# Breakthrough/PySceneDetect

Measured on NVIDIA H100. Metric: frames/sec scored (1080p, ContentDetector), higher is better.
Workload: dtype u8

## Files before the change

### pyscenedetect_b200/csrc/hsv_half2.cuh

```cuda
#pragma once

#include <cuda_fp16.h>
#include <stdint.h>

namespace psd {

struct Px16 {
    uint32_t h[4], s[4], v[4];
};

__device__ __forceinline__ uint32_t y_px(uint32_t b, uint32_t g, uint32_t r) {
    return (r * 4899u + g * 9617u + b * 1868u + 8192u) >> 14;
}

__host__ __device__ constexpr uint32_t y_coef_word(int word, int k0, int which) {
    uint32_t r = 0;
    for (int b = 0; b < 4; ++b) {
        const int g = 4 * word + b - k0;
        uint32_t c = 0;
        if (g == 0) c = which ? 7u : 76u;
        if (g == 1) c = which ? 37u : 145u;
        if (g == 2) c = which ? 19u : 35u;
        r |= c << (8 * b);
    }
    return r;
}

template <int P>
__device__ __forceinline__ uint32_t y_of_pixel(const uint32_t (&w)[12]) {
    constexpr int k0 = 3 * P, j0 = k0 >> 2, j1 = (k0 + 2) >> 2;
    uint32_t lo = __dp4a(w[j0], y_coef_word(j0, k0, 0), 8192u);
    uint32_t hi = __dp4a(w[j0], y_coef_word(j0, k0, 1), 0u);
    if (j1 != j0) {
        lo = __dp4a(w[j1], y_coef_word(j1, k0, 0), lo);
        hi = __dp4a(w[j1], y_coef_word(j1, k0, 1), hi);
    }
    return (hi * 256u + lo) >> 14;
}

__device__ __forceinline__ uint32_t byte_of(const uint32_t (&w)[12], int k) {
    return (w[k >> 2] >> ((k & 3) * 8)) & 0xFFu;
}

struct LutView7 {
    uint32_t cs;
    uint32_t ch;
};

__device__ __forceinline__ LutView7 make_lut7(uint32_t lut_smem_addr, int lane) {
    LutView7 l;
    l.cs = lut_smem_addr + (uint32_t)lane * 4u - 0x6400u * 128u;
    l.ch = lut_smem_addr + 32768u + (uint32_t)lane * 4u;
    return l;
}

__device__ __forceinline__ void lut_fill7(float* lut, int tid, int nthreads) {
    for (int t = tid; t < 512; t += nthreads) {
        const int row = t >> 1, which = t & 1;
        float v = 0.0f;
        if (row) {
            const int q = which ? __double2int_rn(737280.0 / (6.0 * (double)row))
                                : __double2int_rn(1044480.0 / (double)row);
            v = (float)q * 0.000244140625f;
        }
        float4* dst = reinterpret_cast<float4*>(lut + which * 8192 + row * 32);
#pragma unroll
        for (int j = 0; j < 8; ++j) dst[j] = make_float4(v, v, v, v);
    }
}

namespace v7 {

__device__ __forceinline__ __half2 as_h2(uint32_t u) { return *reinterpret_cast<__half2*>(&u); }
__device__ __forceinline__ uint32_t as_u32(__half2 h) { return *reinterpret_cast<uint32_t*>(&h); }

__device__ __forceinline__ uint32_t hsub2u(uint32_t a, uint32_t b) { return as_u32(__hsub2(as_h2(a), as_h2(b))); }
__device__ __forceinline__ uint32_t hfma2u(uint32_t a, uint32_t b, uint32_t c) {
    return as_u32(__hfma2(as_h2(a), as_h2(b), as_h2(c)));
}
__device__ __forceinline__ uint32_t heq2m(uint32_t a, uint32_t b) { return __heq2_mask(as_h2(a), as_h2(b)); }
__device__ __forceinline__ uint32_t bitsel(uint32_t m, uint32_t x, uint32_t y) {
    uint32_t r;
    asm("lop3.b32 %0, %1, %2, %3, 0xCA;" : "=r"(r) : "r"(m), "r"(x), "r"(y));
    return r;
}
__device__ __forceinline__ uint32_t even_bytes_magic(uint32_t t) {
    uint32_t r;
    asm("lop3.b32 %0, %1, 0x00FF00FF, %2, 0xEA;" : "=r"(r) : "r"(t), "r"(0x64006400u));
    return r;
}
__device__ __forceinline__ float lds(uint32_t addr) {
    float r;
    asm volatile("ld.shared.f32 %0, [%1];" : "=f"(r) : "r"(addr));
    return r;
}
__device__ __forceinline__ float fma_rz_(float a, float b, float c) {
    float r;
    asm("fma.rz.f32 %0, %1, %2, %3;" : "=f"(r) : "f"(a), "f"(b), "f"(c));
    return r;
}
__device__ __forceinline__ float fma_rm_(float a, float b, float c) {
    float r;
    asm("fma.rm.f32 %0, %1, %2, %3;" : "=f"(r) : "f"(a), "f"(b), "f"(c));
    return r;
}

struct PairOut7 {
    uint32_t yh0, yh1, ys0, ys1;
    uint32_t vh;
};

__device__ __forceinline__ void pair(uint32_t Bh, uint32_t Gh, uint32_t Rh, const LutView7& lut, PairOut7& o) {
    const uint32_t Vh = __vimax3_u16x2(Bh, Gh, Rh);
    const uint32_t mh = __vimin3_u16x2(Bh, Gh, Rh);
    const uint32_t dh = hsub2u(Vh, mh);
    const uint32_t di = Vh - mh;
    const uint32_t hR = hsub2u(Gh, Bh);
    const uint32_t hG = hfma2u(dh, 0x40004000u, hsub2u(Bh, Rh));
    const uint32_t hB = hfma2u(dh, 0x44004400u, hsub2u(Rh, Gh));
    const uint32_t eR = heq2m(Vh, Rh);
    const uint32_t eG = heq2m(Vh, Gh);
    const uint32_t hh = bitsel(eR, hR, bitsel(eG, hG, hB));
    const float d0 = __low2float(as_h2(dh)), d1 = __high2float(as_h2(dh));
    const float h0 = __low2float(as_h2(hh)), h1 = __high2float(as_h2(hh));
    const uint32_t aS0 = __dp2a_lo(Vh, 0x00000080u, lut.cs), aS1 = __dp2a_lo(Vh, 0x00008000u, lut.cs);
    const uint32_t aH0 = __dp2a_lo(di, 0x00000080u, lut.ch), aH1 = __dp2a_lo(di, 0x00008000u, lut.ch);
    o.ys0 = __float_as_uint(fma_rz_(d0, lds(aS0), 32768.5f));
    o.ys1 = __float_as_uint(fma_rz_(d1, lds(aS1), 32768.5f));
    o.yh0 = __float_as_uint(fma_rm_(h0, lds(aH0), 49152.5f));
    o.yh1 = __float_as_uint(fma_rm_(h1, lds(aH1), 49152.5f));
    o.vh = Vh;
}

__device__ __forceinline__ uint32_t fix_hue4(uint32_t hw) {
    uint32_t m;
    asm("lop3.b32 %0, %1, %2, 0x80808080, 0x80;" : "=r"(m) : "r"(hw), "r"(hw + hw));
    return hw - (m >> 7) * 76u;
}

}

__device__ __forceinline__ void hsv16_v7(const uint32_t (&w)[12], Px16& o, const LutView7& lut) {
    const uint32_t K = 0x64646464u;
#pragma unroll
    for (int g = 0; g < 4; ++g) {
        const uint32_t wa = w[3 * g], wb = w[3 * g + 1], wc = w[3 * g + 2];
        const uint32_t B01 = __byte_perm(wa, K, 0x4340);
        const uint32_t t01 = __byte_perm(wa, wb, 0x5421);
        const uint32_t G01 = v7::even_bytes_magic(t01);
        const uint32_t R01 = __byte_perm(t01, K, 0x4341);
        const uint32_t R23 = __byte_perm(wc, K, 0x4340);
        const uint32_t t23 = __byte_perm(wb, wc, 0x6532);
        const uint32_t B23 = v7::even_bytes_magic(t23);
        const uint32_t G23 = __byte_perm(t23, K, 0x4341);
        v7::PairOut7 p, q;
        v7::pair(B01, G01, R01, lut, p);
        v7::pair(B23, G23, R23, lut, q);
        const uint32_t hw = __byte_perm(__byte_perm(p.yh0, p.yh1, 0x0051), __byte_perm(q.yh0, q.yh1, 0x0051), 0x5410);
        o.h[g] = v7::fix_hue4(hw);
        o.s[g] = __byte_perm(__byte_perm(p.ys0, p.ys1, 0x0051), __byte_perm(q.ys0, q.ys1, 0x0051), 0x5410);
        o.v[g] = __byte_perm(p.vh, q.vh, 0x6420);
    }
}

}
```

### pyscenedetect_b200/csrc/score_kernel.cu

```cuda
#include "hsv_half2.cuh"
#include "psd_common.cuh"

namespace psd {

constexpr int kPxPerThread = 16;

__device__ __forceinline__ uint32_t smem_u32(const void* p) {
    return (uint32_t)__cvta_generic_to_shared(p);
}
__device__ __forceinline__ void mbar_init(unsigned long long* bar, uint32_t count) {
    asm volatile("mbarrier.init.shared::cta.b64 [%0], %1;" ::"r"(smem_u32(bar)), "r"(count));
}
__device__ __forceinline__ void mbar_expect_tx(unsigned long long* bar, uint32_t bytes) {
    asm volatile("mbarrier.arrive.expect_tx.shared::cta.b64 _, [%0], %1;" ::"r"(smem_u32(bar)),
                 "r"(bytes)
                 : "memory");
}
__device__ __forceinline__ void bulk_g2s(void* dst, const void* src, uint32_t bytes,
                                         unsigned long long* bar) {
    asm volatile(
        "cp.async.bulk.shared::cluster.global.mbarrier::complete_tx::bytes [%0], [%1], %2, [%3];" ::
            "r"(smem_u32(dst)),
        "l"(src), "r"(bytes), "r"(smem_u32(bar))
        : "memory");
}

constexpr int kWsConsumerWarps = 24;
constexpr int kWsConsumers = kWsConsumerWarps * 32;
constexpr int kWsStages = 4;
constexpr int kWsSideWarps = kWsStages;
constexpr int kWsThreads = kWsConsumers + kWsSideWarps * 32;
static_assert(kWsSideWarps == 4 && kWsConsumerWarps % 4 == 0, "one side warp per SM sub-partition");
constexpr int kWsUnroll = 4;
constexpr int kWsStripPx = kWsConsumers * kPxPerThread;
constexpr int kWsStripBytes = kWsStripPx * 3;
static_assert(kWsStages % kWsUnroll == 0, "the stage ring must be a whole number of loop bodies");

struct __align__(128) WsSmem {
    uint8_t ring[kWsStages][kWsStripBytes];
    float lut[256 * 64];
    unsigned long long full[kWsStages];
    unsigned long long empty[kWsStages];
    uint32_t accl[kWsStages][4][32];
    uint32_t accl_sink[kWsStages][4][32];
    uint32_t yhist[kWsStages][256];
    uint32_t vhist[kWsStages][256];
};

__device__ __forceinline__ uint32_t sad4_acc(uint32_t a, uint32_t b, uint32_t c) {
    uint32_t r;
    asm volatile("vabsdiff4.u32.u32.u32.add %0, %1, %2, %3;" : "=r"(r) : "r"(a), "r"(b), "r"(c));
    return r;
}
template <int OFF>
__device__ __forceinline__ void mbar_wait_hint_off(uint32_t bar, uint32_t parity) {
    asm volatile(
        "{\n\t"
        ".reg .pred p;\n\t"
        "WAIT_%=:\n\t"
        "mbarrier.try_wait.parity.shared::cta.b64 p, [%0+%3], %1, %2;\n\t"
        "@p bra DONE_%=;\n\t"
        "bra WAIT_%=;\n\t"
        "DONE_%=:\n\t"
        "}" ::"r"(bar),
        "r"(parity), "r"(20000u), "n"(OFF)
        : "memory");
}
__device__ __forceinline__ void mbar_wait_hint(unsigned long long* bar, uint32_t parity) {
    mbar_wait_hint_off<0>(smem_u32(bar), parity);
}
template <int OFF>
__device__ __forceinline__ void lds128_off(uint32_t addr, uint32_t& x, uint32_t& y, uint32_t& z, uint32_t& w) {
    asm volatile("ld.shared.v4.u32 {%0,%1,%2,%3}, [%4+%5];" : "=r"(x), "=r"(y), "=r"(z), "=r"(w) : "r"(addr), "n"(OFF));
}
template <int OFF>
__device__ __forceinline__ void red_shared_add_off(uint32_t addr, uint32_t v) {
    asm volatile("red.shared.add.u32 [%0+%2], %1;" ::"r"(addr), "r"(v), "n"(OFF) : "memory");
}
template <int OFF>
__device__ __forceinline__ void mbar_arrive_off(uint32_t bar) {
    asm volatile("mbarrier.arrive.shared::cta.b64 _, [%0+%1];" ::"r"(bar), "n"(OFF) : "memory");
}

__host__ __device__ __forceinline__ int chunk_first(int c, int n_frames, int n_chunks) {
    return (int)(((long long)c * n_frames) / n_chunks);
}
struct WsItem {
    int f0, nf;
    int px0, valid_px;
    int it_begin;
    int slots;
    int walked;
};
__device__ __forceinline__ WsItem ws_item(const ScoreArgs& a, int item) {
    WsItem w;
    const int chunk = item % a.n_chunks;
    const int strip = item / a.n_chunks;
    w.f0 = chunk_first(chunk, a.n_frames, a.n_chunks);
    w.nf = chunk_first(chunk + 1, a.n_frames, a.n_chunks) - w.f0;
    w.px0 = strip * kWsStripPx;
    w.valid_px = min(kWsStripPx, a.n_pixels - w.px0) & ~15;
    const bool have_halo = (a.features & PSD_F_HSV) && (w.f0 > 0 || a.prev != nullptr);
    w.it_begin = have_halo ? 0 : 1;
    w.walked = w.nf + 1 - w.it_begin;
    w.slots = (w.walked + kWsUnroll - 1) / kWsUnroll * kWsUnroll;
    return w;
}

struct WsAddr {
    uint32_t ring;
    uint32_t full;
    uint32_t acc;
};

template <uint32_t F, int J>
__device__ __forceinline__ void ws_step(const ScoreArgs& a, WsSmem& sm, const WsAddr& ad, uint32_t parity, int stage0,
                                        uint32_t sad_acc, bool mine, int fi, int my_px, int lane, uint32_t zero,
                                        const LutView7& lut7, const Px16& prev, Px16& cur) {
    constexpr bool kHSV = (F & PSD_F_HSV) != 0;
    constexpr bool kSUM = (F & PSD_F_BGRSUM) != 0;
    constexpr bool kYH = (F & PSD_F_YHIST) != 0;
    constexpr bool kEDGE = (F & PSD_F_EDGES) != 0;
    if (kHSV) {
        if ((J & 1) == 0) {
            mbar_wait_hint_off<J * 8>(ad.full, parity);
            mbar_wait_hint_off<J * 8 + 8>(ad.full, parity);
        }
    } else {
        mbar_wait_hint_off<J * 8>(ad.full, parity);
    }
    uint32_t w[12];
    lds128_off<J * kWsStripBytes>(ad.ring, w[0], w[1], w[2], w[3]);
    lds128_off<J * kWsStripBytes + 16>(ad.ring, w[4], w[5], w[6], w[7]);
    lds128_off<J * kWsStripBytes + 32>(ad.ring, w[8], w[9], w[10], w[11]);
    if (kHSV) {
        hsv16_v7(w, cur, lut7);
        uint32_t sad_h = sad4_acc(cur.h[0], prev.h[0], zero), sad_s = sad4_acc(cur.s[0], prev.s[0], zero),
                 sad_v = sad4_acc(cur.v[0], prev.v[0], zero);
#pragma unroll
        for (int j = 1; j < 4; ++j) {
            sad_h = sad4_acc(cur.h[j], prev.h[j], sad_h);
            sad_s = sad4_acc(cur.s[j], prev.s[j], sad_s);
            sad_v = sad4_acc(cur.v[j], prev.v[j], sad_v);
        }
        red_shared_add_off<J * 512>(sad_acc, sad_h);
        red_shared_add_off<J * 512 + 128>(sad_acc, sad_s);
        red_shared_add_off<J * 512 + 256>(sad_acc, sad_v);
        if (kEDGE && mine) {
            uint8_t* vp = a.vplane + (int64_t)fi * a.n_pixels + my_px;
            if ((a.n_pixels & 15) == 0) {
                *reinterpret_cast<uint4*>(vp) = make_uint4(cur.v[0], cur.v[1], cur.v[2], cur.v[3]);
            } else {
                for (int p = 0; p < kPxPerThread; ++p) vp[p] = (uint8_t)(cur.v[p >> 2] >> ((p & 3) * 8));
            }
            const uint32_t vh = smem_u32(sm.vhist[stage0 + J]);
#pragma unroll
            for (int p = 0; p < kPxPerThread; ++p)
                red_shared_add_off<0>(__dp4a(cur.v[p >> 2], 4u << ((p & 3) * 8), vh), 1u);
        }
    }
    if (mine) {
        if (kSUM) {
            uint32_t bsum = 0;
#pragma unroll
            for (int j = 0; j < 12; ++j) bsum = __dp4a(w[j], 0x01010101u, bsum);
            red_shared_add_off<J * 512 + 384>(ad.acc, bsum);
        }
        if (kYH) {
            uint32_t* hist = sm.yhist[stage0 + J];
#define PSD_YH(i) atomicAdd(&hist[y_of_pixel<i>(w)], 1u);
            PSD_YH(0) PSD_YH(1) PSD_YH(2) PSD_YH(3) PSD_YH(4) PSD_YH(5) PSD_YH(6) PSD_YH(7)
            PSD_YH(8) PSD_YH(9) PSD_YH(10) PSD_YH(11) PSD_YH(12) PSD_YH(13) PSD_YH(14) PSD_YH(15)
#undef PSD_YH
        }
    }
    if (lane == 0) mbar_arrive_off<kWsStages * 8 + J * 8>(ad.full);
}

template <int J>
__device__ __forceinline__ void ws_null_step(const WsAddr& ad, uint32_t parity, int lane) {
    mbar_wait_hint_off<J * 8>(ad.full, parity);
    if (lane == 0) mbar_arrive_off<kWsStages * 8 + J * 8>(ad.full);
}

template <uint32_t F>
__global__ void __launch_bounds__(kWsThreads, 1) psd_score_ws_kernel(const ScoreArgs a) {
    extern __shared__ __align__(128) uint8_t smem_raw[];
    WsSmem& sm = *reinterpret_cast<WsSmem*>(smem_raw);
    constexpr bool kHSV = (F & PSD_F_HSV) != 0;
    constexpr bool kSUM = (F & PSD_F_BGRSUM) != 0;
    constexpr bool kYH = (F & PSD_F_YHIST) != 0;
    constexpr bool kEDGE = (F & PSD_F_EDGES) != 0;
    constexpr int U = kWsUnroll;

    const int tid = threadIdx.x;
    const int lane = tid & 31;
    const int n_items = a.n_chunks * a.n_strips;

    for (int i = tid; i < kWsStages * 256; i += kWsThreads) {
        (&sm.yhist[0][0])[i] = 0;
        (&sm.vhist[0][0])[i] = 0;
    }
    for (int i = tid; i < kWsStages * 4 * 32; i += kWsThreads) {
        (&sm.accl[0][0][0])[i] = 0;
        (&sm.accl_sink[0][0][0])[i] = 0;
    }
    if (kHSV) lut_fill7(sm.lut, tid, kWsThreads);
    if (tid == 0) {
        for (int s = 0; s < kWsStages; ++s) {
            mbar_init(&sm.full[s], 1);
            mbar_init(&sm.empty[s], kWsConsumerWarps);
        }
        asm volatile("fence.mbarrier_init.release.cluster;" ::: "memory");
    }
    __syncthreads();

    if (tid >= kWsConsumers) {
        struct Cursor {
            int item, slot;
            WsItem w;
        };
        const int rs = (tid - kWsConsumers) >> 5;
        auto load = [&](Cursor& c) { if (c.item < n_items) c.w = ws_item(a, c.item); };
        auto advance = [&](Cursor& c) {
            c.slot += kWsStages;
            if (c.slot >= c.w.slots) { c.slot = rs; c.item += gridDim.x; load(c); }
        };
        auto issue = [&](Cursor& c) {
            if (lane == 0) {
                if (c.slot < c.w.walked) {
                    const int fi = c.w.f0 - 1 + c.w.it_begin + c.slot;
                    const uint8_t* src = (fi < 0 ? a.prev : a.frames + (int64_t)fi * a.frame_stride) + (int64_t)c.w.px0 * 3;
                    const uint32_t bytes = (uint32_t)c.w.valid_px * 3u;
                    mbar_expect_tx(&sm.full[rs], bytes);
                    bulk_g2s(sm.ring[rs], src, bytes, &sm.full[rs]);
                } else {
                    mbar_arrive_off<0>(smem_u32(&sm.full[rs]));
                }
            }
            advance(c);
        };
        Cursor ret{(int)blockIdx.x, rs, {}};
        load(ret);
        Cursor iss = ret;
        issue(iss);
        uint32_t parity = 0;
        while (ret.item < n_items) {
            mbar_wait_hint(&sm.empty[rs], parity);
            const int it = ret.w.it_begin + ret.slot;
            const bool real = ret.slot < ret.w.walked;
            const bool own = real && it >= 1;
            const int fi = ret.w.f0 - 1 + it;
            uint32_t tot[4] = {0u, 0u, 0u, 0u};
            if (own && (kHSV || kSUM)) {
#pragma unroll
                for (int c = 0; c < 4; ++c) {
                    if ((c < 3 && kHSV) || (c == 3 && kSUM)) {
                        tot[c] = sm.accl[rs][c][lane];
                        sm.accl[rs][c][lane] = 0;
                    }
                }
            }
            if (own) {
                if (kYH) {
#pragma unroll
                    for (int b = lane; b < 256; b += 32) {
                        const uint32_t v = sm.yhist[rs][b];
                        if (v) { sm.yhist[rs][b] = 0; atomicAdd(&a.yhist[(int64_t)fi * 256 + b], v); }
                    }
                }
                if (kEDGE) {
#pragma unroll
                    for (int b = lane; b < 256; b += 32) {
                        const uint32_t v = sm.vhist[rs][b];
                        if (v) { sm.vhist[rs][b] = 0; atomicAdd(&a.vhist[(int64_t)fi * 256 + b], v); }
                    }
                }
                if (ret.item < a.n_chunks && lane == 0)
                    a.sums[fi].has_prev = (fi > 0 || a.prev != nullptr) ? 1ull : 0ull;
            }
            __syncwarp();
            if (iss.item < n_items) issue(iss);
            if (own && (kHSV || kSUM)) {
#pragma unroll
                for (int c = 0; c < 4; ++c) {
                    if ((c < 3 && !kHSV) || (c == 3 && !kSUM)) continue;
                    const uint32_t v = __reduce_add_sync(0xFFFFFFFFu, tot[c]);
                    if (lane == 0 && v)
                        atomicAdd(reinterpret_cast<unsigned long long*>(&a.sums[fi]) + (c < 3 ? c : 4),
                                  (unsigned long long)v);
                }
            }
            advance(ret);
            parity ^= 1u;
        }
        return;
    }

    const LutView7 lut7 = make_lut7(smem_u32(sm.lut), lane);
    const uint32_t zero = a.shift24 ^ 0x01000000u;
    const uint32_t ring0 = smem_u32(sm.ring[0]) + tid * 48;
    const uint32_t full0 = smem_u32(&sm.full[0]);
    const uint32_t accl0 = smem_u32(&sm.accl[0][0][lane]);
    const uint32_t sink0 = smem_u32(&sm.accl_sink[0][0][lane]);
    int stage0 = 0;
    uint32_t parity = 0;
    WsAddr ad{ring0, full0, 0u};
    auto next_body = [&](uint32_t acc0) {
        stage0 += U;
        if (stage0 == kWsStages) {
            stage0 = 0;
            parity ^= 1u;
            ad.ring = ring0; ad.full = full0; ad.acc = acc0;
        } else {
            ad.ring += U * kWsStripBytes; ad.full += U * 8; ad.acc += U * 512;
        }
    };
    for (int item = blockIdx.x; item < n_items; item += gridDim.x) {
        const WsItem wi = ws_item(a, item);
        const int my_px = wi.px0 + tid * kPxPerThread;
        const bool active = tid * kPxPerThread < wi.valid_px;
        const uint32_t acc0 = active ? accl0 : sink0;
        ad.acc = acc0 + stage0 * 512;
        Px16 P0, P1;
#pragma unroll
        for (int j = 0; j < 4; ++j) P0.h[j] = P0.s[j] = P0.v[j] = P1.h[j] = P1.s[j] = P1.v[j] = 0;
        const int n = wi.walked;
        const int fbase = wi.f0 - 1 + wi.it_begin;
        int k = 0;
        uint32_t acc_first = sink0 + stage0 * 512;
#pragma unroll 1
        for (; k + U <= n; k += U) {
            const bool first_mine = active && (wi.it_begin + k >= 1);
            ws_step<F, 0>(a, sm, ad, parity, stage0, acc_first, first_mine, fbase + k, my_px, lane, zero, lut7, P0, P1);
            ws_step<F, 1>(a, sm, ad, parity, stage0, ad.acc, active, fbase + k + 1, my_px, lane, zero, lut7, P1, P0);
            ws_step<F, 2>(a, sm, ad, parity, stage0, ad.acc, active, fbase + k + 2, my_px, lane, zero, lut7, P0, P1);
            ws_step<F, 3>(a, sm, ad, parity, stage0, ad.acc, active, fbase + k + 3, my_px, lane, zero, lut7, P1, P0);
            next_body(acc0);
            acc_first = ad.acc;
        }
        if (k < n) {
            const int r = n - k;
            ws_step<F, 0>(a, sm, ad, parity, stage0, acc_first, active && (wi.it_begin + k >= 1), fbase + k, my_px,
                              lane, zero, lut7, P0, P1);
            if (r > 1) ws_step<F, 1>(a, sm, ad, parity, stage0, ad.acc, active, fbase + k + 1, my_px, lane, zero, lut7, P1, P0);
            else ws_null_step<1>(ad, parity, lane);
            if (r > 2) ws_step<F, 2>(a, sm, ad, parity, stage0, ad.acc, active, fbase + k + 2, my_px, lane, zero, lut7, P0, P1);
            else ws_null_step<2>(ad, parity, lane);
            ws_null_step<3>(ad, parity, lane);
            next_body(acc0);
        }
    }
}

static int pick_chunks(int n_frames, int n_strips, int grid) {
    long long best_cost = -1;
    int best = 1;
    const int c_max = n_frames < 4096 ? n_frames : 4096;
    for (int c = 1; c <= c_max; ++c) {
        const int longest = (n_frames + c - 1) / c;
        if (longest < 8 && c > 1) break;
        const long long per_cta = ((long long)n_strips * c + grid - 1) / grid;
        const long long cost = per_cta * (longest + 1);
        if (best_cost < 0 || cost < best_cost) { best_cost = cost; best = c; }
    }
    return best;
}

template <uint32_t F>
static int launch_ws(ScoreArgs a, int n_ws_strips, cudaStream_t stream) {
    const int smem = (int)sizeof(WsSmem);
    static int sm_count = 0;
    if (sm_count == 0) {
        int dev = 0;
        PSD_CUDA(cudaGetDevice(&dev));
        PSD_CUDA(cudaDeviceGetAttribute(&sm_count, cudaDevAttrMultiProcessorCount, dev));
    }
    PSD_CUDA(cudaFuncSetAttribute(psd_score_ws_kernel<F>, cudaFuncAttributeMaxDynamicSharedMemorySize, smem));
    a.shift24 = 0x01000000u;
    a.features = F;
    a.n_strips = n_ws_strips;
    a.n_chunks = pick_chunks(a.n_frames, n_ws_strips, sm_count);
    if (a.n_chunks > a.n_frames) a.n_chunks = a.n_frames;
    const int64_t items = (int64_t)a.n_chunks * n_ws_strips;
    PSD_REQUIRE(items > 0 && items < 2147483647LL, "score work items out of range (%lld)", (long long)items);
    const int grid = (int)(items < sm_count ? items : sm_count);
    psd_score_ws_kernel<F><<<grid, kWsThreads, smem, stream>>>(a);
    PSD_CHECK_LAUNCH();
    count_launch();
    return PSD_OK;
}

static int dispatch_ws(const ScoreArgs& a, uint32_t f, int n_ws_strips, cudaStream_t s) {
    switch (f & 15u) {
#define CASE(F) case F: return launch_ws<F>(a, n_ws_strips, s);
        CASE(1) CASE(2) CASE(3) CASE(4) CASE(5) CASE(6) CASE(7)
        CASE(9) CASE(11) CASE(13) CASE(15)
#undef CASE
        default:
            set_error("unsupported feature mask 0x%x", f);
            return PSD_ERR_INVALID;
    }
}

constexpr int kTailThreads = 128;
constexpr int kLutBytes = 256 * 64 * 4;

__device__ __forceinline__ void load_tail(const uint8_t* src, int n_bytes, uint32_t (&w)[12]) {
#pragma unroll
    for (int j = 0; j < 12; ++j) w[j] = 0;
#pragma unroll
    for (int k = 0; k < 48; ++k)
        if (k < n_bytes) w[k >> 2] |= (uint32_t)src[k] << ((k & 3) * 8);
}

__global__ void __launch_bounds__(kTailThreads) psd_score_tail_kernel(const ScoreArgs a) {
    extern __shared__ __align__(128) float lut[];
    const bool hsv = (a.features & PSD_F_HSV) != 0;
    if (hsv) lut_fill7(lut, threadIdx.x, blockDim.x);
    __syncthreads();
    const int fi = blockIdx.x * blockDim.x + threadIdx.x;
    if (fi >= a.n_frames) return;
    const int p16 = a.n_pixels & ~15, n = a.n_pixels - p16;
    const uint8_t* prev = fi > 0 ? a.frames + (int64_t)(fi - 1) * a.frame_stride : a.prev;
    uint32_t w[12];
    load_tail(a.frames + (int64_t)fi * a.frame_stride + (int64_t)p16 * 3, 3 * n, w);
    unsigned long long* sums = reinterpret_cast<unsigned long long*>(&a.sums[fi]);
    if (hsv) {
        const LutView7 lut7 = make_lut7(smem_u32(lut), threadIdx.x & 31);
        Px16 cur;
        hsv16_v7(w, cur, lut7);
        if (prev) {
            uint32_t wp[12];
            load_tail(prev + (int64_t)p16 * 3, 3 * n, wp);
            Px16 pre;
            hsv16_v7(wp, pre, lut7);
            uint32_t sad_h = 0, sad_s = 0, sad_v = 0;
#pragma unroll
            for (int j = 0; j < 4; ++j) {
                sad_h = __vsadu4(cur.h[j], pre.h[j]) + sad_h;
                sad_s = __vsadu4(cur.s[j], pre.s[j]) + sad_s;
                sad_v = __vsadu4(cur.v[j], pre.v[j]) + sad_v;
            }
            atomicAdd(sums + 0, (unsigned long long)sad_h);
            atomicAdd(sums + 1, (unsigned long long)sad_s);
            atomicAdd(sums + 2, (unsigned long long)sad_v);
        }
        if (a.features & PSD_F_EDGES) {
            uint8_t* vp = a.vplane + (int64_t)fi * a.n_pixels + p16;
            for (int p = 0; p < n; ++p) {
                const uint32_t v = (cur.v[p >> 2] >> ((p & 3) * 8)) & 0xFFu;
                vp[p] = (uint8_t)v;
                atomicAdd(&a.vhist[(int64_t)fi * 256 + v], 1u);
            }
        }
    }
    if (a.features & PSD_F_BGRSUM) {
        uint32_t bsum = 0;
#pragma unroll
        for (int j = 0; j < 12; ++j) bsum = __dp4a(w[j], 0x01010101u, bsum);
        atomicAdd(sums + 4, (unsigned long long)bsum);
    }
    if (a.features & PSD_F_YHIST) {
        for (int p = 0; p < n; ++p)
            atomicAdd(&a.yhist[(int64_t)fi * 256 + y_px(byte_of(w, 3 * p), byte_of(w, 3 * p + 1), byte_of(w, 3 * p + 2))],
                      1u);
    }
    if (p16 == 0) a.sums[fi].has_prev = (fi > 0 || a.prev != nullptr) ? 1ull : 0ull;
}

static int launch_tail(ScoreArgs a, uint32_t features, cudaStream_t stream) {
    PSD_CUDA(cudaFuncSetAttribute(psd_score_tail_kernel, cudaFuncAttributeMaxDynamicSharedMemorySize, kLutBytes));
    a.features = features;
    const int grid = (a.n_frames + kTailThreads - 1) / kTailThreads;
    psd_score_tail_kernel<<<grid, kTailThreads, (features & PSD_F_HSV) ? kLutBytes : 0, stream>>>(a);
    PSD_CHECK_LAUNCH();
    count_launch();
    return PSD_OK;
}

int launch_score(const ScoreArgs& a, uint32_t features, cudaStream_t stream) {
    if (features & PSD_F_EDGES) features |= PSD_F_HSV;
    PSD_REQUIRE(a.n_frames > 0 && a.n_pixels > 0, "empty score launch");
    const uintptr_t al = reinterpret_cast<uintptr_t>(a.frames) | (uintptr_t)a.frame_stride |
                         reinterpret_cast<uintptr_t>(a.prev);
    PSD_REQUIRE((al & 15) == 0, "score pass input is not 16-byte aligned");
    const int p16 = a.n_pixels & ~15;
    if (p16 > 0) {
        const int rc = dispatch_ws(a, features, (p16 + kWsStripPx - 1) / kWsStripPx, stream);
        if (rc) return rc;
    }
    if (p16 < a.n_pixels) return launch_tail(a, features, stream);
    return PSD_OK;
}

__global__ void psd_test_hsv_kernel(const uint8_t* bgr, int64_t n_groups, uint8_t* h, uint8_t* s,
                                    uint8_t* v, uint8_t* y) {
    extern __shared__ __align__(128) float lutmem[];
    lut_fill7(lutmem, threadIdx.x, blockDim.x);
    const LutView7 lut7 = make_lut7(smem_u32(lutmem), threadIdx.x & 31);
    __syncthreads();
    for (int64_t g = blockIdx.x * (int64_t)blockDim.x + threadIdx.x; g < n_groups;
         g += (int64_t)gridDim.x * blockDim.x) {
        uint32_t w[12];
        const uint4* p = reinterpret_cast<const uint4*>(bgr + g * 48);
        const uint4 q0 = p[0], q1 = p[1], q2 = p[2];
        w[0] = q0.x; w[1] = q0.y; w[2] = q0.z; w[3] = q0.w;
        w[4] = q1.x; w[5] = q1.y; w[6] = q1.z; w[7] = q1.w;
        w[8] = q2.x; w[9] = q2.y; w[10] = q2.z; w[11] = q2.w;
        Px16 o;
        hsv16_v7(w, o, lut7);
        *reinterpret_cast<uint4*>(h + g * 16) = make_uint4(o.h[0], o.h[1], o.h[2], o.h[3]);
        *reinterpret_cast<uint4*>(s + g * 16) = make_uint4(o.s[0], o.s[1], o.s[2], o.s[3]);
        *reinterpret_cast<uint4*>(v + g * 16) = make_uint4(o.v[0], o.v[1], o.v[2], o.v[3]);
        for (int px = 0; px < 16; ++px)
            y[g * 16 + px] = (uint8_t)y_px(byte_of(w, 3 * px), byte_of(w, 3 * px + 1), byte_of(w, 3 * px + 2));
    }
}

}

extern "C" int psd_test_hsv(int device, const uint8_t* bgr_host, int64_t n_pixels, uint8_t* h_out,
                            uint8_t* s_out, uint8_t* v_out, uint8_t* y_out) {
    using namespace psd;
    PSD_REQUIRE(n_pixels > 0 && (n_pixels % 16) == 0, "n_pixels must be a positive multiple of 16");
    PSD_CUDA(cudaSetDevice(device));
    int sm_count = 0;
    PSD_CUDA(cudaDeviceGetAttribute(&sm_count, cudaDevAttrMultiProcessorCount, device));
    uint8_t *d_bgr = nullptr, *d_out = nullptr;
    PSD_CUDA(cudaMalloc(&d_bgr, (size_t)n_pixels * 3));
    PSD_CUDA(cudaMalloc(&d_out, (size_t)n_pixels * 4));
    PSD_CUDA(cudaMemcpy(d_bgr, bgr_host, (size_t)n_pixels * 3, cudaMemcpyHostToDevice));
    uint8_t* dh = d_out;
    uint8_t* ds = d_out + n_pixels;
    uint8_t* dv = d_out + 2 * n_pixels;
    uint8_t* dy = d_out + 3 * n_pixels;
    PSD_CUDA(cudaFuncSetAttribute(psd_test_hsv_kernel, cudaFuncAttributeMaxDynamicSharedMemorySize, kLutBytes));
    psd_test_hsv_kernel<<<sm_count * 2, 256, kLutBytes>>>(d_bgr, n_pixels / 16, dh, ds, dv, dy);
    PSD_CHECK_LAUNCH();
    count_launch();
    PSD_CUDA(cudaDeviceSynchronize());
    PSD_CUDA(cudaMemcpy(h_out, dh, (size_t)n_pixels, cudaMemcpyDeviceToHost));
    PSD_CUDA(cudaMemcpy(s_out, ds, (size_t)n_pixels, cudaMemcpyDeviceToHost));
    PSD_CUDA(cudaMemcpy(v_out, dv, (size_t)n_pixels, cudaMemcpyDeviceToHost));
    PSD_CUDA(cudaMemcpy(y_out, dy, (size_t)n_pixels, cudaMemcpyDeviceToHost));
    cudaFree(d_bgr);
    cudaFree(d_out);
    return PSD_OK;
}
```

Before: 505,800.

## Prefetch next ring stage into registers midway through HSV conversion

For the HSV-only consumer path, each step now waits on the next stage's mbarrier and loads the next strip into a second register buffer halfway through the HSV conversion. This hides shared-memory load latency and barrier waits behind arithmetic. The stage ring is fixed to one lap per loop body, which drops the stage0 bookkeeping and the next_body address updates. In exchange it uses more registers for the double buffer and adds more complex parity and tail handling.

```diff
diff --git a/pyscenedetect_b200/csrc/hsv_half2.cuh b/pyscenedetect_b200/csrc/hsv_half2.cuh
--- a/pyscenedetect_b200/csrc/hsv_half2.cuh
+++ b/pyscenedetect_b200/csrc/hsv_half2.cuh
@@ -140,10 +140,11 @@
 
 }
 
-__device__ __forceinline__ void hsv16_v7(const uint32_t (&w)[12], Px16& o, const LutView7& lut) {
+template <int G0, int G1>
+__device__ __forceinline__ void hsv_groups_v7(const uint32_t (&w)[12], Px16& o, const LutView7& lut) {
     const uint32_t K = 0x64646464u;
 #pragma unroll
-    for (int g = 0; g < 4; ++g) {
+    for (int g = G0; g < G1; ++g) {
         const uint32_t wa = w[3 * g], wb = w[3 * g + 1], wc = w[3 * g + 2];
         const uint32_t B01 = __byte_perm(wa, K, 0x4340);
         const uint32_t t01 = __byte_perm(wa, wb, 0x5421);
@@ -163,4 +164,8 @@
     }
 }
 
+__device__ __forceinline__ void hsv16_v7(const uint32_t (&w)[12], Px16& o, const LutView7& lut) {
+    hsv_groups_v7<0, 4>(w, o, lut);
 }
+
+}
diff --git a/pyscenedetect_b200/csrc/score_kernel.cu b/pyscenedetect_b200/csrc/score_kernel.cu
--- a/pyscenedetect_b200/csrc/score_kernel.cu
+++ b/pyscenedetect_b200/csrc/score_kernel.cu
@@ -34,7 +34,7 @@
 constexpr int kWsUnroll = 4;
 constexpr int kWsStripPx = kWsConsumers * kPxPerThread;
 constexpr int kWsStripBytes = kWsStripPx * 3;
-static_assert(kWsStages % kWsUnroll == 0, "the stage ring must be a whole number of loop bodies");
+static_assert(kWsStages == kWsUnroll, "a consumer loop body is one lap of the stage ring");
 
 struct __align__(128) WsSmem {
     uint8_t ring[kWsStages][kWsStripBytes];
@@ -113,28 +113,52 @@
     uint32_t acc;
 };
 
+template <int J>
+__device__ __forceinline__ void ws_load(const WsAddr& ad, uint32_t (&w)[12]) {
+    lds128_off<J * kWsStripBytes>(ad.ring, w[0], w[1], w[2], w[3]);
+    lds128_off<J * kWsStripBytes + 16>(ad.ring, w[4], w[5], w[6], w[7]);
+    lds128_off<J * kWsStripBytes + 32>(ad.ring, w[8], w[9], w[10], w[11]);
+}
+
+__host__ __device__ constexpr bool ws_looks_ahead(uint32_t f) {
+    return (f & PSD_F_HSV) && !(f & (PSD_F_BGRSUM | PSD_F_YHIST));
+}
+
+template <int J>
+__device__ __forceinline__ void ws_look_ahead(const WsAddr& ad, uint32_t parity, bool more, uint32_t (&wn)[12]) {
+    if (J == kWsStages - 1) {
+        if (more) {
+            mbar_wait_hint_off<0>(ad.full, parity ^ 1u);
+            ws_load<0>(ad, wn);
+        }
+    } else {
+        mbar_wait_hint_off<J * 8 + 8>(ad.full, parity);
+        ws_load<J + 1>(ad, wn);
+    }
+}
+
 template <uint32_t F, int J>
-__device__ __forceinline__ void ws_step(const ScoreArgs& a, WsSmem& sm, const WsAddr& ad, uint32_t parity, int stage0,
-                                        uint32_t sad_acc, bool mine, int fi, int my_px, int lane, uint32_t zero,
-                                        const LutView7& lut7, const Px16& prev, Px16& cur) {
+__device__ __forceinline__ void ws_step(const ScoreArgs& a, WsSmem& sm, const WsAddr& ad, uint32_t parity,
+                                        uint32_t sad_acc, bool mine, bool more, int fi, int my_px, int lane,
+                                        uint32_t zero, const LutView7& lut7, const Px16& prev, Px16& cur,
+                                        uint32_t (&w)[12], uint32_t (&wn)[12]) {
     constexpr bool kHSV = (F & PSD_F_HSV) != 0;
     constexpr bool kSUM = (F & PSD_F_BGRSUM) != 0;
     constexpr bool kYH = (F & PSD_F_YHIST) != 0;
     constexpr bool kEDGE = (F & PSD_F_EDGES) != 0;
+    if (!ws_looks_ahead(F)) {
+        if (!kHSV || (J & 1) == 0) mbar_wait_hint_off<J * 8>(ad.full, parity);
+        if (kHSV && (J & 1) == 0) mbar_wait_hint_off<J * 8 + 8>(ad.full, parity);
+        ws_load<J>(ad, w);
+    }
     if (kHSV) {
-        if ((J & 1) == 0) {
-            mbar_wait_hint_off<J * 8>(ad.full, parity);
-            mbar_wait_hint_off<J * 8 + 8>(ad.full, parity);
-        }
-    } else {
-        mbar_wait_hint_off<J * 8>(ad.full, parity);
-    }
-    uint32_t w[12];
-    lds128_off<J * kWsStripBytes>(ad.ring, w[0], w[1], w[2], w[3]);
-    lds128_off<J * kWsStripBytes + 16>(ad.ring, w[4], w[5], w[6], w[7]);
-    lds128_off<J * kWsStripBytes + 32>(ad.ring, w[8], w[9], w[10], w[11]);
-    if (kHSV) {
-        hsv16_v7(w, cur, lut7);
+        if (ws_looks_ahead(F)) {
+            hsv_groups_v7<0, 2>(w, cur, lut7);
+            ws_look_ahead<J>(ad, parity, more, wn);
+            hsv_groups_v7<2, 4>(w, cur, lut7);
+        } else {
+            hsv16_v7(w, cur, lut7);
+        }
         uint32_t sad_h = sad4_acc(cur.h[0], prev.h[0], zero), sad_s = sad4_acc(cur.s[0], prev.s[0], zero),
                  sad_v = sad4_acc(cur.v[0], prev.v[0], zero);
 #pragma unroll
@@ -153,7 +177,7 @@
             } else {
                 for (int p = 0; p < kPxPerThread; ++p) vp[p] = (uint8_t)(cur.v[p >> 2] >> ((p & 3) * 8));
             }
-            const uint32_t vh = smem_u32(sm.vhist[stage0 + J]);
+            const uint32_t vh = smem_u32(sm.vhist[J]);
 #pragma unroll
             for (int p = 0; p < kPxPerThread; ++p)
                 red_shared_add_off<0>(__dp4a(cur.v[p >> 2], 4u << ((p & 3) * 8), vh), 1u);
@@ -167,7 +191,7 @@
             red_shared_add_off<J * 512 + 384>(ad.acc, bsum);
         }
         if (kYH) {
-            uint32_t* hist = sm.yhist[stage0 + J];
+            uint32_t* hist = sm.yhist[J];
 #define PSD_YH(i) atomicAdd(&hist[y_of_pixel<i>(w)], 1u);
             PSD_YH(0) PSD_YH(1) PSD_YH(2) PSD_YH(3) PSD_YH(4) PSD_YH(5) PSD_YH(6) PSD_YH(7)
             PSD_YH(8) PSD_YH(9) PSD_YH(10) PSD_YH(11) PSD_YH(12) PSD_YH(13) PSD_YH(14) PSD_YH(15)
@@ -299,56 +323,56 @@
 
     const LutView7 lut7 = make_lut7(smem_u32(sm.lut), lane);
     const uint32_t zero = a.shift24 ^ 0x01000000u;
-    const uint32_t ring0 = smem_u32(sm.ring[0]) + tid * 48;
-    const uint32_t full0 = smem_u32(&sm.full[0]);
     const uint32_t accl0 = smem_u32(&sm.accl[0][0][lane]);
     const uint32_t sink0 = smem_u32(&sm.accl_sink[0][0][lane]);
-    int stage0 = 0;
     uint32_t parity = 0;
-    WsAddr ad{ring0, full0, 0u};
-    auto next_body = [&](uint32_t acc0) {
-        stage0 += U;
-        if (stage0 == kWsStages) {
-            stage0 = 0;
-            parity ^= 1u;
-            ad.ring = ring0; ad.full = full0; ad.acc = acc0;
-        } else {
-            ad.ring += U * kWsStripBytes; ad.full += U * 8; ad.acc += U * 512;
-        }
-    };
+    WsAddr ad{smem_u32(sm.ring[0]) + tid * 48, smem_u32(&sm.full[0]), 0u};
+    uint32_t wa[12], wb[12];
+    if (ws_looks_ahead(F)) {
+        mbar_wait_hint_off<0>(ad.full, parity);
+        ws_load<0>(ad, wa);
+    }
     for (int item = blockIdx.x; item < n_items; item += gridDim.x) {
         const WsItem wi = ws_item(a, item);
         const int my_px = wi.px0 + tid * kPxPerThread;
         const bool active = tid * kPxPerThread < wi.valid_px;
-        const uint32_t acc0 = active ? accl0 : sink0;
-        ad.acc = acc0 + stage0 * 512;
+        ad.acc = active ? accl0 : sink0;
+        const bool next_item = item + (int)gridDim.x < n_items;
         Px16 P0, P1;
 #pragma unroll
         for (int j = 0; j < 4; ++j) P0.h[j] = P0.s[j] = P0.v[j] = P1.h[j] = P1.s[j] = P1.v[j] = 0;
         const int n = wi.walked;
         const int fbase = wi.f0 - 1 + wi.it_begin;
         int k = 0;
-        uint32_t acc_first = sink0 + stage0 * 512;
+        uint32_t acc_first = sink0;
 #pragma unroll 1
         for (; k + U <= n; k += U) {
             const bool first_mine = active && (wi.it_begin + k >= 1);
-            ws_step<F, 0>(a, sm, ad, parity, stage0, acc_first, first_mine, fbase + k, my_px, lane, zero, lut7, P0, P1);
-            ws_step<F, 1>(a, sm, ad, parity, stage0, ad.acc, active, fbase + k + 1, my_px, lane, zero, lut7, P1, P0);
-            ws_step<F, 2>(a, sm, ad, parity, stage0, ad.acc, active, fbase + k + 2, my_px, lane, zero, lut7, P0, P1);
-            ws_step<F, 3>(a, sm, ad, parity, stage0, ad.acc, active, fbase + k + 3, my_px, lane, zero, lut7, P1, P0);
-            next_body(acc0);
+            const bool more = k + U < n || next_item;
+            ws_step<F, 0>(a, sm, ad, parity, acc_first, first_mine, more, fbase + k, my_px, lane, zero, lut7, P0, P1,
+                          wa, wb);
+            ws_step<F, 1>(a, sm, ad, parity, ad.acc, active, more, fbase + k + 1, my_px, lane, zero, lut7, P1, P0,
+                          wb, wa);
+            ws_step<F, 2>(a, sm, ad, parity, ad.acc, active, more, fbase + k + 2, my_px, lane, zero, lut7, P0, P1,
+                          wa, wb);
+            ws_step<F, 3>(a, sm, ad, parity, ad.acc, active, more, fbase + k + 3, my_px, lane, zero, lut7, P1, P0,
+                          wb, wa);
+            parity ^= 1u;
             acc_first = ad.acc;
         }
         if (k < n) {
             const int r = n - k;
-            ws_step<F, 0>(a, sm, ad, parity, stage0, acc_first, active && (wi.it_begin + k >= 1), fbase + k, my_px,
-                              lane, zero, lut7, P0, P1);
-            if (r > 1) ws_step<F, 1>(a, sm, ad, parity, stage0, ad.acc, active, fbase + k + 1, my_px, lane, zero, lut7, P1, P0);
+            ws_step<F, 0>(a, sm, ad, parity, acc_first, active && (wi.it_begin + k >= 1), next_item, fbase + k, my_px,
+                          lane, zero, lut7, P0, P1, wa, wb);
+            if (r > 1) ws_step<F, 1>(a, sm, ad, parity, ad.acc, active, next_item, fbase + k + 1, my_px, lane, zero,
+                                     lut7, P1, P0, wb, wa);
             else ws_null_step<1>(ad, parity, lane);
-            if (r > 2) ws_step<F, 2>(a, sm, ad, parity, stage0, ad.acc, active, fbase + k + 2, my_px, lane, zero, lut7, P0, P1);
+            if (r > 2) ws_step<F, 2>(a, sm, ad, parity, ad.acc, active, next_item, fbase + k + 2, my_px, lane, zero,
+                                     lut7, P0, P1, wa, wb);
             else ws_null_step<2>(ad, parity, lane);
             ws_null_step<3>(ad, parity, lane);
-            next_body(acc0);
+            if (ws_looks_ahead(F)) ws_look_ahead<3>(ad, parity, next_item, wa);
+            parity ^= 1u;
         }
     }
 }
```

Result: no change. 506,600, median of 6 (+0.2%).
